# MiksuNy/rust_ray_tracing

Measured on AMD Instinct MI355X. Metric: Mray/s at 1920x1080, 8 spp, Sponza BVH; 1/2/4/8-GPU scaling + % HBM roofline, higher is better.
Workload: dtype f32

## Files before the change

include/mipt_diag.h:

```cpp
#ifndef MIPT_DIAG_H
#define MIPT_DIAG_H

#include <stdint.h>

#ifdef __cplusplus
extern "C" {
#endif

#if defined(__GNUC__)
#define MIPT_DIAG_API __attribute__((visibility("default")))
#else
#define MIPT_DIAG_API
#endif

MIPT_DIAG_API int mipt_debug_eval(int op, const float *a, const float *b, uint64_t n, float *out);

MIPT_DIAG_API int mipt_debug_eval_range(int op, uint32_t first_bits, uint64_t n, float y, float *out);

MIPT_DIAG_API int mipt_debug_wgsl(int op, const float *in, uint64_t n, const uint32_t *texels, uint32_t tex_w, uint32_t tex_h, float *out);

MIPT_DIAG_API int mipt_debug_texel(const float *uv, uint64_t n, const uint32_t *pool, uint64_t pool_words, uint32_t offset, uint32_t w, uint32_t h,
                                   float *rgb_out, uint64_t *clamped_out);

MIPT_DIAG_API int mipt_debug_divide(float *d_buf, uint64_t n_floats, float divisor, void *stream);
MIPT_DIAG_API int mipt_debug_popcount(const uint32_t *d_bitmap, uint64_t n_words, uint64_t *d_out, void *stream);

MIPT_DIAG_API int mipt_debug_tile_order(const uint32_t *cost, uint32_t n_tiles, uint32_t samples, uint32_t *order_out);
MIPT_DIAG_API int mipt_diag_scene_tile_order(const void *scene, uint32_t *cost_out, uint32_t *order_out, uint32_t cap, uint32_t info_out[3]);

MIPT_DIAG_API int mipt_debug_hot_select(const uint32_t *cost, uint32_t n_slots, uint32_t samples, uint32_t n_hot, uint32_t *hot_out, uint32_t *bits_out);
MIPT_DIAG_API int mipt_diag_scene_hot_pixels(const void *scene, uint32_t *pixel_cost_out, uint32_t cap_slots, uint32_t *hot_out, uint32_t cap_hot, uint32_t info_out[3]);

MIPT_DIAG_API const char *mipt_diag_last_error(void);

MIPT_DIAG_API int mipt_internal_pair_order(const void *nodes, uint32_t n_nodes, uint32_t *order_out, uint32_t cap, uint32_t *n_records_out);
MIPT_DIAG_API uint32_t mipt_internal_pair_order_top(void);
MIPT_DIAG_API int mipt_internal_tri_slots(const void *nodes, uint32_t n_nodes, uint32_t n_tris, uint32_t *slot_out, uint32_t *n_slots_out);

MIPT_DIAG_API int mipt_diag_scene_sizes(const void *scene, uint64_t out[2]);
MIPT_DIAG_API int mipt_diag_scene_tables(const void *scene, uint64_t out[3]);
MIPT_DIAG_API int mipt_diag_scene_read(const void *scene, int which, void *dst, uint64_t bytes);
MIPT_DIAG_API int mipt_diag_scene_hash(const void *scene, uint64_t out[2]);

MIPT_DIAG_API int mipt_diag_host_layout(const void *desc, uint8_t *geom_out, uint64_t geom_cap, uint8_t *attr_out, uint64_t attr_cap,
                                        uint64_t *sizes_out, uint32_t *info_out);

MIPT_DIAG_API int mipt_diag_hash_words(const void *words, uint64_t n_words, uint64_t *out);

MIPT_DIAG_API int mipt_diag_write_obj(const char *path, const void *tris, uint64_t n_tris, const char *mtllib, const char *const *material_names,
                                      uint32_t n_materials);

#ifdef __cplusplus
}
#endif
#endif
```

rust_ray_tracing_amd/_lib.py:

```python
from __future__ import annotations

import ctypes as C
import os

import numpy as np

_HERE = os.path.dirname(os.path.abspath(__file__))
LIB_PATH = os.environ.get("MIPT_LIB") or os.path.join(_HERE, "libmipt.so")

VERTEX = np.dtype([("position", "<f4", 3), ("tex_coord_x", "<f4"), ("normal", "<f4", 3), ("tex_coord_y", "<f4")])
TRIANGLE = np.dtype([("vertices", VERTEX, 3), ("material_id", "<u4"), ("_pad", "u1", 12)])
NODE = np.dtype([("bounds_min", "<f4", 3), ("first_tri_or_child", "<u4"), ("bounds_max", "<f4", 3), ("num_tris", "<u4")])
MATERIAL = np.dtype([
    ("base_color", "<f4", 3), ("transmission", "<f4"), ("specular_tint", "<f4", 3), ("ior", "<f4"),
    ("emission", "<f4", 3), ("roughness", "<f4"), ("metallic", "<f4"), ("transparency", "<f4"),
    ("base_color_tex_id", "<u4"), ("transparency_tex_id", "<u4"), ("roughness_tex_id", "<u4"),
    ("metallic_tex_id", "<u4"), ("emission_tex_id", "<u4"), ("normal_tex_id", "<u4")])
CAMERA = np.dtype([("look_at", "<f4", (4, 4)), ("position", "<f4", 3), ("_pad", "<f4")])
assert VERTEX.itemsize == 32 and TRIANGLE.itemsize == 112 and NODE.itemsize == 32
assert MATERIAL.itemsize == 80 and CAMERA.itemsize == 80

NO_TEXTURE = 0xFFFFFFFF

SEED_PIXEL_STREAM, SEED_PER_SAMPLE = 0, 1
# ... 348 lines not shown
    lib.mipt_temporal_history_bytes.argtypes = [u32, u32, u32]
    lib.mipt_temporal_history_bytes.restype = u64
    lib.mipt_temporal.argtypes = [to, vp, tb, C.c_int]
    lib.mipt_temporal.restype = C.c_int
    lib.mipt_temporal_device.argtypes = [to, vp, tb, vp]
    lib.mipt_temporal_device.restype = C.c_int
    vo, vb = C.POINTER(MiptVarianceOptions), C.POINTER(MiptVarianceBuffers)
    lib.mipt_denoise_variance_workspace_bytes.argtypes = [u32, u32, u32]
    lib.mipt_denoise_variance_workspace_bytes.restype = u64
    lib.mipt_denoise_variance.argtypes = [vo, vb, C.c_int]
    lib.mipt_denoise_variance.restype = C.c_int
    lib.mipt_denoise_variance_device.argtypes = [vo, vb, vp, u64, vp]
    lib.mipt_denoise_variance_device.restype = C.c_int
    uo, ub = C.POINTER(MiptUpsampleOptions), C.POINTER(MiptUpsampleBuffers)
    lib.mipt_upsample_workspace_bytes.argtypes = [u32, u32, u32, u32]
    lib.mipt_upsample_workspace_bytes.restype = u64
    lib.mipt_upsample.argtypes = [uo, ub, C.c_int]
    lib.mipt_upsample.restype = C.c_int
    lib.mipt_upsample_device.argtypes = [uo, ub, vp, u64, vp]
    lib.mipt_upsample_device.restype = C.c_int
    lib.mipt_render_adaptive.argtypes = [vp, vp, u32, C.POINTER(MiptOptions), vp, vp, vp, C.POINTER(MiptStats)]
    lib.mipt_render_adaptive.restype = C.c_int
    lib.mipt_render_adaptive_device.argtypes = [vp, vp, u32, C.POINTER(MiptOptions), vp, vp, vp, vp, C.POINTER(MiptStats)]
    lib.mipt_render_adaptive_device.restype = C.c_int
    so, sb = C.POINTER(MiptSampleMapOptions), C.POINTER(MiptSampleMapBuffers)
    lib.mipt_sample_map_workspace_bytes.argtypes = [u32, u32, u32]
    lib.mipt_sample_map_workspace_bytes.restype = u64
    lib.mipt_sample_map.argtypes = [so, sb, C.c_int]
    lib.mipt_sample_map.restype = C.c_int
    lib.mipt_sample_map_device.argtypes = [so, sb, vp, vp]
    lib.mipt_sample_map_device.restype = C.c_int
    return lib


MULTITEST_LIB_PATH = os.path.join(_HERE, "libmipt_multitest.so")
_multitest = None


def load_multitest() -> C.CDLL:
    global _multitest
    if _multitest is not None:
        return _multitest
    load()
    if not os.path.exists(MULTITEST_LIB_PATH):
        raise ImportError(f"{MULTITEST_LIB_PATH} is missing: run __graft_entry__.build()")
    lib = _bind(C.CDLL(MULTITEST_LIB_PATH))
    lib.rccl_double_inject.argtypes = [C.c_int, C.c_int]
    lib.rccl_double_inject.restype = C.c_longlong
    _multitest = lib
    return lib


DIAG_LIB_PATH = os.path.join(_HERE, "libmipt_diag.so")
DIAG_EXPORTS = ["mipt_debug_eval", "mipt_debug_eval_range", "mipt_debug_wgsl", "mipt_debug_texel", "mipt_debug_divide", "mipt_debug_popcount", "mipt_debug_tile_order", "mipt_diag_scene_tile_order", "mipt_debug_hot_select", "mipt_diag_scene_hot_pixels", "mipt_diag_last_error",
                "mipt_internal_pair_order", "mipt_internal_pair_order_top", "mipt_internal_tri_slots",
                "mipt_diag_scene_sizes", "mipt_diag_scene_tables", "mipt_diag_scene_read", "mipt_diag_scene_hash", "mipt_diag_write_obj", "mipt_diag_host_layout", "mipt_diag_hash_words"]
_diag = None


def load_diag() -> C.CDLL:
    global _diag
    if _diag is not None:
        return _diag
    load()
    if not os.path.exists(DIAG_LIB_PATH):
        raise ImportError(f"{DIAG_LIB_PATH} is missing: run __graft_entry__.build()")
    lib = C.CDLL(DIAG_LIB_PATH)
    vp = C.c_void_p
    lib.mipt_debug_eval.argtypes = [C.c_int, vp, vp, C.c_uint64, vp]
    lib.mipt_debug_eval.restype = C.c_int
    lib.mipt_debug_eval_range.argtypes = [C.c_int, C.c_uint32, C.c_uint64, C.c_float, vp]
    lib.mipt_debug_eval_range.restype = C.c_int
    lib.mipt_debug_wgsl.argtypes = [C.c_int, vp, C.c_uint64, vp, C.c_uint32, C.c_uint32, vp]
    lib.mipt_debug_wgsl.restype = C.c_int
    lib.mipt_debug_texel.argtypes = [vp, C.c_uint64, vp, C.c_uint64, C.c_uint32, C.c_uint32, C.c_uint32, vp, C.POINTER(C.c_uint64)]
    lib.mipt_debug_texel.restype = C.c_int
    lib.mipt_debug_divide.argtypes = [vp, C.c_uint64, C.c_float, vp]
    lib.mipt_debug_divide.restype = C.c_int
    lib.mipt_debug_popcount.argtypes = [vp, C.c_uint64, vp, vp]
    lib.mipt_debug_popcount.restype = C.c_int
    lib.mipt_debug_tile_order.argtypes = [vp, C.c_uint32, C.c_uint32, vp]
    lib.mipt_debug_tile_order.restype = C.c_int
    lib.mipt_diag_scene_tile_order.argtypes = [vp, vp, vp, C.c_uint32, C.POINTER(C.c_uint32 * 3)]
    lib.mipt_diag_scene_tile_order.restype = C.c_int
    lib.mipt_debug_hot_select.argtypes = [vp, C.c_uint32, C.c_uint32, C.c_uint32, vp, vp]
    lib.mipt_debug_hot_select.restype = C.c_int
    lib.mipt_diag_scene_hot_pixels.argtypes = [vp, vp, C.c_uint32, vp, C.c_uint32, C.POINTER(C.c_uint32 * 3)]
    lib.mipt_diag_scene_hot_pixels.restype = C.c_int
    lib.mipt_diag_last_error.argtypes = []
    lib.mipt_diag_last_error.restype = C.c_char_p
    u32p = C.POINTER(C.c_uint32)
    lib.mipt_internal_pair_order.argtypes = [vp, C.c_uint32, vp, C.c_uint32, u32p]
    lib.mipt_internal_pair_order.restype = C.c_int
    lib.mipt_internal_pair_order_top.argtypes = []
    lib.mipt_internal_pair_order_top.restype = C.c_uint32
    lib.mipt_internal_tri_slots.argtypes = [vp, C.c_uint32, C.c_uint32, vp, u32p]
    lib.mipt_internal_tri_slots.restype = C.c_int
    lib.mipt_diag_scene_sizes.argtypes = [vp, C.POINTER(C.c_uint64 * 2)]
    lib.mipt_diag_scene_sizes.restype = C.c_int
    lib.mipt_diag_scene_tables.argtypes = [vp, C.POINTER(C.c_uint64 * 3)]
    lib.mipt_diag_scene_tables.restype = C.c_int
    lib.mipt_diag_scene_read.argtypes = [vp, C.c_int, vp, C.c_uint64]
    lib.mipt_diag_scene_read.restype = C.c_int
    lib.mipt_diag_scene_hash.argtypes = [vp, C.POINTER(C.c_uint64 * 2)]
    lib.mipt_diag_scene_hash.restype = C.c_int
    lib.mipt_diag_write_obj.argtypes = [C.c_char_p, vp, C.c_uint64, C.c_char_p, C.POINTER(C.c_char_p), C.c_uint32]
    lib.mipt_diag_write_obj.restype = C.c_int
    lib.mipt_diag_host_layout.argtypes = [vp, vp, C.c_uint64, vp, C.c_uint64, C.POINTER(C.c_uint64 * 2), C.POINTER(C.c_uint32 * 4)]
    lib.mipt_diag_host_layout.restype = C.c_int
    lib.mipt_diag_hash_words.argtypes = [vp, C.c_uint64, C.POINTER(C.c_uint64)]
    lib.mipt_diag_hash_words.restype = C.c_int
    _diag = lib
    return lib


class MiptError(RuntimeError):
    def __init__(self, code: int, where: str):
        self.code = code
        msg = load().mipt_last_error()
        super().__init__(f"{where} failed with status {code}: {msg.decode() if msg else ''}")


def check(code: int, where: str) -> None:
    if code != 0:
        raise MiptError(code, where)


def ptr(a: np.ndarray) -> C.c_void_p:
    return C.c_void_p(a.ctypes.data)
```

rust_ray_tracing_amd/csrc/mipt_api.cpp:

```cpp
#include "../../include/mipt.h"
#include "pt_kernel.h"
#include "mipt_scene.h"

#include <atomic>
#include <chrono>
#include <cmath>
#include <cstdarg>
#include <cstdio>
#include <cstdlib>
#include <cstring>
#include <exception>
#include <memory>
#include <mutex>
#include <new>
#include <string>
#include <thread>
#include <vector>

static_assert(sizeof(MiptVec3) == 12, "Vec3f");
static_assert(sizeof(MiptVertex) == 32, "Vertex");
static_assert(sizeof(MiptTriangle) == 112 && offsetof(MiptTriangle, material_id) == 96, "Triangle");
static_assert(sizeof(MiptNode) == 32 && offsetof(MiptNode, first_tri_or_child) == 12 &&
                  offsetof(MiptNode, bounds_max) == 16 && offsetof(MiptNode, num_tris) == 28, "Node");
static_assert(sizeof(MiptMaterial) == 80 && offsetof(MiptMaterial, ior) == 28 && offsetof(MiptMaterial, emission) == 32 &&
// ... 397 lines not shown
    if (nodes_cap < scene->n_nodes) return fail(MIPT_ERR_INVALID_ARG, "mipt_scene_get_bvh: nodes_cap %u < %u nodes", nodes_cap, scene->n_nodes);
    MIPT_HIP(hipSetDevice(scene->device));
    MIPT_HIP(hipMemcpy(nodes_out, scene->d_nodes, (size_t)scene->n_nodes * sizeof(MiptNode), hipMemcpyDeviceToHost));
    if (tri_order_out) MIPT_HIP(hipMemcpy(tri_order_out, scene->d_tri_order, scene->n_tris * sizeof(uint32_t), hipMemcpyDeviceToHost));
    if (n_nodes_out) *n_nodes_out = scene->n_nodes;
    return MIPT_OK;
}

uint64_t mipt_packed_pixels(uint32_t width, uint32_t height, uint32_t tile_world) {
    if (tile_world == 0) tile_world = 1;
    const uint64_t tiles = (uint64_t)((width + 7u) / 8u) * ((height + 7u) / 8u);
    return ((tiles + tile_world - 1u) / tile_world) * 64ull;
}

static int validate_options(const MiptOptions *opt) {
    if (!opt) return fail(MIPT_ERR_INVALID_ARG, "options == NULL");
    if (opt->width == 0 || opt->height == 0) return fail(MIPT_ERR_INVALID_ARG, "Width and height must be greater than 0");
    if (opt->max_ray_depth == 0) return fail(MIPT_ERR_INVALID_ARG, "Max ray depth must be greater than 0");
    if (opt->samples == 0) return fail(MIPT_ERR_INVALID_ARG, "Sample count must be greater than 0");
    if ((uint64_t)opt->width * opt->height >= 2147483648ull - 87636354ull)
        return fail(MIPT_ERR_INVALID_ARG, "width*height too large for the reference's 32-bit pixel seed");
    if (opt->seed_mode > MIPT_SEED_PER_SAMPLE) return fail(MIPT_ERR_INVALID_ARG, "unknown seed_mode %u", opt->seed_mode);
    if (opt->traversal > MIPT_TRAVERSAL_CULLED) return fail(MIPT_ERR_INVALID_ARG, "unknown traversal %u", opt->traversal);
    const uint32_t world = opt->tile_world ? opt->tile_world : 1u;
    if (opt->tile_rank >= world) return fail(MIPT_ERR_INVALID_ARG, "tile_rank %u >= tile_world %u", opt->tile_rank, world);
    if ((opt->flags & MIPT_FLAG_SUM) && opt->seed_mode != MIPT_SEED_PER_SAMPLE && opt->sample_begin > 1)
        return fail(MIPT_ERR_INVALID_ARG, "sample_begin needs MIPT_SEED_PER_SAMPLE (the pixel stream cannot be entered mid-way)");
    if (opt->shading > MIPT_SHADING_WGPU) return fail(MIPT_ERR_INVALID_ARG, "unknown shading mode %u", opt->shading);
    if (!(opt->cull_margin >= 0.0f) || opt->cull_margin > 1.0f) return fail(MIPT_ERR_INVALID_ARG, "cull_margin must be in [0, 1]");
    for (uint32_t r : opt->reserved)
        if (r) return fail(MIPT_ERR_INVALID_ARG, "reserved option fields must be 0");
    return MIPT_OK;
}

static int validate_batch(const MiptScene *scene, const MiptCamera *cameras, uint32_t n_views, const MiptOptions *opt, const char *who) {
    if (!scene || !cameras) return fail(MIPT_ERR_INVALID_ARG, "%s: null scene or cameras", who);
    if (n_views == 0) return fail(MIPT_ERR_INVALID_ARG, "%s: n_views == 0", who);
    int rc = validate_options(opt);
    if (rc) return rc;
    if (opt->tile_world > 1) return fail(MIPT_ERR_INVALID_ARG, "%s: tile_world %u: a batch is not tile-sharded (0 or 1)", who, opt->tile_world);
    if (opt->flags & MIPT_FLAG_PACKED) return fail(MIPT_ERR_INVALID_ARG, "%s: MIPT_FLAG_PACKED: a batch is not tile-sharded", who);
    if ((uint64_t)n_views * opt->width * opt->height >= MIPT_BATCH_MAX_PIXELS)
        return fail(MIPT_ERR_INVALID_ARG, "%s: %u views of %ux%u: n_views*width*height must stay below 2^32", who, n_views, opt->width, opt->height);
    return MIPT_OK;
}

}
#ifndef MIPT_HOT_LANES_NUM
#define MIPT_HOT_LANES_NUM 2
#endif
#ifndef MIPT_HOT_LANES_DEN
#define MIPT_HOT_LANES_DEN 1
#endif
static int render_launch(MiptScene *scene, const MiptCamera *cameras, uint32_t n_views, bool batch, const MiptOptions *opt,
                         float *d_hdr_rgb, uint8_t *d_rgba8, void *hip_stream, MiptStats *stats, bool pack_single) {
    const char *who = batch ? "mipt_render_batch_device" : "mipt_render_device";
    int rc = MIPT_OK;
    if (batch) {
        if ((rc = validate_batch(scene, cameras, n_views, opt, who))) return rc;
    } else {
        if (!scene || !cameras) return fail(MIPT_ERR_INVALID_ARG, "mipt_render_device: null scene or camera");
        if ((rc = validate_options(opt))) return rc;
    }
    if (!d_hdr_rgb) return fail(MIPT_ERR_INVALID_ARG, "%s: d_hdr_rgb == NULL", who);
    const uint32_t world = opt->tile_world ? opt->tile_world : 1u;
    const bool packed = (opt->flags & MIPT_FLAG_PACKED) != 0 && (world > 1 || pack_single);
    if ((opt->flags & MIPT_FLAG_ACCUM) && !(opt->flags & MIPT_FLAG_SUM))
        return fail(MIPT_ERR_INVALID_ARG, "MIPT_FLAG_ACCUM needs MIPT_FLAG_SUM (a running sum, divided once at the end)");
    if (d_rgba8 && (packed || (opt->flags & MIPT_FLAG_SUM)))
        return fail(MIPT_ERR_INVALID_ARG, "RGBA8 output needs a full-frame mean buffer (not PACKED / SUM)");
    MIPT_HIP(hipSetDevice(scene->device));
    hipStream_t stream = (hipStream_t)hip_stream;
    const MiptCamera *camera = cameras;

    mipt::DevParams pr{};
    pr.width = opt->width; pr.height = opt->height; pr.samples = opt->samples; pr.max_depth = opt->max_ray_depth;
    pr.seed_mode = opt->shading == MIPT_SHADING_WGPU ? (uint32_t)MIPT_SEED_PER_SAMPLE : opt->seed_mode;
    pr.sample_begin = opt->sample_begin ? opt->sample_begin : 1u;
    pr.sum_only = (opt->flags & MIPT_FLAG_SUM) ? 1u : 0u;
    pr.packed = packed ? 1u : 0u;
    pr.accumulate = (opt->flags & MIPT_FLAG_ACCUM) ? 1u : 0u;
    pr.tile_rank = opt->tile_rank; pr.tile_world = world;
    pr.tiles_x = (opt->width + 7u) / 8u; pr.tiles_y = (opt->height + 7u) / 8u;
    const uint64_t tiles = (uint64_t)pr.tiles_x * pr.tiles_y;
    pr.n_local_tiles = (uint32_t)((tiles + world - 1u - opt->tile_rank) / world);
    pr.total_work = (unsigned long long)pr.n_local_tiles * 64ull * n_views;
    pr.aspect = (float)opt->width / (float)opt->height;
    pr.samples_f = (float)opt->samples;
    pr.cull_scale = 1.0f + opt->cull_margin;
    pr.service_num = 3; pr.service_den = 8; pr.reverse_tiles = 0;
    for (int c = 0; c < 3; c++)
        for (int r = 0; r < 3; r++) pr.cam[c * 3 + r] = camera->look_at[c][r];
    pr.cam[9] = camera->position.x; pr.cam[10] = camera->position.y; pr.cam[11] = camera->position.z;
    pr.hdr = d_hdr_rgb;
    pr.stats = scene->d_stats;

    const bool count = (opt->flags & MIPT_FLAG_COUNT) != 0;
    const bool cull = opt->traversal == MIPT_TRAVERSAL_CULLED;
    const int occ = mipt::trace_blocks_per_cu(batch, count, cull, (int)opt->shading);
    int bpc = occ;
    {
        const long long fit = (long long)(pr.total_work / (unsigned long long)(1.25 * scene->n_cu * mipt::kBlockThreads));
        const int cap = (int)(fit < 2 ? 2 : fit);
        if (cap < bpc) bpc = cap;
    }
    pr.leaf_period = (pr.total_work >= 4ull * (unsigned long long)scene->n_cu * (unsigned long long)occ * mipt::kBlockThreads) ? 4u : 1u;
    pr.leaf_den = 4u;
    int grid = 0;
    if ((rc = mipt::traversal_grid(scene, bpc, pr.total_work, &grid))) return rc;
    pr.ovf = scene->d_ovf;

    const bool touched = count && (opt->flags & MIPT_FLAG_TOUCHED) != 0 && opt->shading == 0;
    const size_t geom_lines = ((size_t)scene->dev.geom_bytes + 127) / 128, attr_lines = (scene->n_tris + 1) / 2;
    const size_t geom_words = (geom_lines + 31) / 32, attr_words = (attr_lines + 31) / 32;
    pr.touched = nullptr; pr.touched_attr_base = (uint32_t)(geom_words * 32);
    if (touched) {
        if (!scene->d_touched) MIPT_HIP(hipMalloc((void **)&scene->d_touched, (geom_words + attr_words) * sizeof(uint32_t)));
        MIPT_HIP(hipMemsetAsync(scene->d_touched, 0, (geom_words + attr_words) * sizeof(uint32_t), stream));
        pr.touched = scene->d_touched;
    }
    const bool order_on = !count && !batch && opt->shading == MIPT_SHADING_CPU && !(opt->flags & MIPT_FLAG_ACCUM) && pr.n_local_tiles != 0u &&
                          pr.n_local_tiles < (1u << 26);
    pr.tile_order = nullptr; pr.pixel_cost = nullptr; pr.hot = nullptr; pr.hot_bits = nullptr; pr.n_hot = 0u;
    const uint32_t n_slots = order_on ? pr.n_local_tiles * 64u : 0u;
    uint32_t hot_next = 0u;
    if (order_on) {
        const unsigned long long lanes = (unsigned long long)grid * mipt::kBlockThreads * MIPT_HOT_LANES_NUM / MIPT_HOT_LANES_DEN;
        hot_next = (uint32_t)(lanes < n_slots / 4u ? lanes : n_slots / 4u);
    }
    if (order_on) {
        const uint32_t key[7] = {opt->width, opt->height, world, opt->tile_rank, pr.n_local_tiles, pr.seed_mode, opt->samples};
        const size_t bytes = (size_t)pr.n_local_tiles * sizeof(uint32_t);
        const size_t hot_bytes = (size_t)(n_slots / 4u) * sizeof(uint32_t), work_bytes = mipt::hot_work_words(n_slots) * sizeof(uint32_t);
        if (scene->tile_cost_bytes < bytes || scene->tile_order_bytes < bytes || scene->pixel_cost_bytes < bytes * 64 || scene->hot_bytes < hot_bytes ||
            scene->hot_bits_bytes < bytes * 2 || scene->hot_work_bytes < work_bytes || memcmp(key, scene->tile_key, sizeof key) != 0 ||
            memcmp(pr.cam, scene->tile_cam, sizeof pr.cam) != 0)
            scene->tile_order_valid = false;
        if ((rc = mipt::grow_device_buffer((void **)&scene->d_tile_cost, &scene->tile_cost_bytes, bytes))) return rc;
        if ((rc = mipt::grow_device_buffer((void **)&scene->d_tile_order, &scene->tile_order_bytes, bytes))) return rc;
        if ((rc = mipt::grow_device_buffer((void **)&scene->d_pixel_cost, &scene->pixel_cost_bytes, bytes * 64))) return rc;
        if ((rc = mipt::grow_device_buffer((void **)&scene->d_hot, &scene->hot_bytes, hot_bytes))) return rc;
        if ((rc = mipt::grow_device_buffer((void **)&scene->d_hot_bits, &scene->hot_bits_bytes, bytes * 2))) return rc;
        if ((rc = mipt::grow_device_buffer((void **)&scene->d_hot_work, &scene->hot_work_bytes, work_bytes))) return rc;
        memcpy(scene->tile_key, key, sizeof key);
        memcpy(scene->tile_cam, pr.cam, sizeof pr.cam);
        MIPT_HIP(hipMemsetAsync(scene->d_pixel_cost, 0, bytes * 64, stream));
        pr.pixel_cost = scene->d_pixel_cost;
        pr.tile_order = scene->tile_order_valid ? scene->d_tile_order : nullptr;
        scene->tile_order_used = scene->tile_order_valid;
        scene->hot_used = 0u;
        if (scene->tile_order_valid && scene->hot_n != 0u) {
            pr.hot = scene->d_hot; pr.hot_bits = scene->d_hot_bits; pr.n_hot = scene->hot_n;
            pr.total_work += scene->hot_n;
            scene->hot_used = scene->hot_n;
        }
        scene->tile_order_valid = false;
    }
    mipt::DevBatch bt{};
    if (batch) {
        scene->h_cams.assign((size_t)n_views * 4, make_float4(0.0f, 0.0f, 0.0f, 0.0f));
        for (uint32_t v = 0; v < n_views; v++) {
            const MiptCamera &c = cameras[v];
            for (int col = 0; col < 3; col++) scene->h_cams[(size_t)v * 4 + col] = make_float4(c.look_at[col][0], c.look_at[col][1], c.look_at[col][2], 0.0f);
            scene->h_cams[(size_t)v * 4 + 3] = make_float4(c.position.x, c.position.y, c.position.z, 0.0f);
        }
        const size_t bytes = scene->h_cams.size() * sizeof(float4);
        if ((rc = mipt::grow_device_buffer((void **)&scene->d_cams, &scene->cams_bytes, bytes))) return rc;
        MIPT_HIP(hipMemcpyAsync(scene->d_cams, scene->h_cams.data(), bytes, hipMemcpyHostToDevice, stream));
        bt.cams = scene->d_cams;
        bt.view_pixels = opt->width * opt->height;
        bt.tiles_recip = 0xffffffffu / pr.n_local_tiles;
    }
    mipt::DevStats hs;
    float ms = 0.0f;
    rc = mipt::traversal_launch(
        scene, stream,
        [&]() -> int {
            MIPT_HIP(mipt::launch_trace(scene->dev, pr, batch ? &bt : nullptr, count, cull, (int)opt->shading, (int)grid, stream));
            return MIPT_OK;
        },
        [&]() -> int {
            if (order_on) {
                MIPT_HIP(mipt::launch_pixel_reduce(scene->d_pixel_cost, n_slots, opt->samples, scene->d_tile_cost, scene->d_hot_work, stream));
                MIPT_HIP(mipt::launch_tile_order(scene->d_tile_cost, pr.n_local_tiles, opt->samples, scene->d_tile_order, stream));
                if (hot_next != 0u)
                    MIPT_HIP(mipt::launch_hot_select(scene->d_pixel_cost, n_slots, opt->samples, hot_next, scene->d_hot_work, scene->d_hot, scene->d_hot_bits, stream));
                scene->hot_n = hot_next;
                scene->tile_order_valid = true;
            }
            if (touched) {
                MIPT_HIP(mipt::launch_popcount(scene->d_touched, geom_words, &scene->d_stats->touched_geom, stream));
                MIPT_HIP(mipt::launch_popcount(scene->d_touched + geom_words, attr_words, &scene->d_stats->touched_attr, stream));
            }
            if (d_rgba8) MIPT_HIP(mipt::launch_tonemap(d_hdr_rgb, (unsigned long long)opt->width * opt->height * n_views, 1.0f, d_rgba8, stream));
            return MIPT_OK;
        },
        hs, ms);
    if (rc && rc != MIPT_ERR_STACK) return rc;
    if (stats) {
        memset(stats, 0, sizeof *stats);
        stats->kernel_ms = ms;
        stats->rays = hs.rays; stats->inner_steps = hs.inner_steps; stats->tri_tests = hs.tri_tests;
        stats->hits = hs.hits; stats->texel_fetches = hs.texel_fetches; stats->stack_overflows = hs.stack_overflows;
        stats->tex_clamped = hs.tex_clamped; stats->max_stack = hs.max_stack; stats->pixels = hs.pixels;
        stats->diag[0] = hs.d_iters; stats->diag[1] = hs.d_inner_lanes; stats->diag[2] = hs.d_leaf_lanes;
        stats->diag[3] = hs.d_iters_inner; stats->diag[4] = hs.d_iters_leaf; stats->diag[5] = hs.d_services;
        stats->diag[6] = hs.d_service_lanes; stats->diag[7] = hs.d_cycles_service; stats->diag[8] = hs.d_cycles_total; stats->diag[9] = hs.d_cycles_mem; stats->diag[10] = hs.d_cycles_tail;
        stats->touched_lines[0] = hs.touched_geom; stats->touched_lines[1] = hs.touched_attr;
    }
    return rc;
}

int mipt::check_batch_args(const MiptScene *scene, const MiptCamera *cameras, uint32_t n_views, const MiptOptions *opt, const char *who) {
    return validate_batch(scene, cameras, n_views, opt, who);
}

int mipt::render_device_impl(MiptScene *scene, const MiptCamera *camera, const MiptOptions *opt,
                             float *d_hdr_rgb, uint8_t *d_rgba8, void *hip_stream, MiptStats *stats, bool pack_single) {
    return render_launch(scene, camera, 1u, false, opt, d_hdr_rgb, d_rgba8, hip_stream, stats, pack_single);
}

extern "C" {

int mipt_render_batch_device(MiptScene *scene, const MiptCamera *cameras, uint32_t n_views, const MiptOptions *opt,
                             float *d_hdr_rgb, uint8_t *d_rgba8, void *hip_stream, MiptStats *stats) {
    MIPT_NO_THROW(render_launch(scene, cameras, n_views, true, opt, d_hdr_rgb, d_rgba8, hip_stream, stats, false))
}

int mipt_render_batch(MiptScene *scene, const MiptCamera *cameras, uint32_t n_views, const MiptOptions *opt,
                      float *hdr_rgb, uint8_t *rgba8, MiptStats *stats) {
    int rc = validate_batch(scene, cameras, n_views, opt, "mipt_render_batch");
    if (rc) return rc;
    if (opt->flags & MIPT_FLAG_ACCUM) return fail(MIPT_ERR_INVALID_ARG, "MIPT_FLAG_ACCUM needs a caller-owned device buffer: use mipt_render_batch_device");
    if (rgba8 && (opt->flags & MIPT_FLAG_SUM))
        return fail(MIPT_ERR_INVALID_ARG, "RGBA8 output needs a full-frame mean buffer (not PACKED / SUM)");
    MIPT_HIP(hipSetDevice(scene->device));
    const uint64_t n_pix = (uint64_t)n_views * opt->width * opt->height;
    if ((rc = mipt::grow_device_buffer((void **)&scene->d_hdr, &scene->hdr_bytes, (size_t)n_pix * 3 * sizeof(float)))) return rc;
    uint8_t *d_rgba = nullptr;
    if (rgba8) {
// ... 88 lines not shown
```

rust_ray_tracing_amd/csrc/mipt_diag.hip:

```cpp
#include "../../include/mipt_diag.h"
#include "pt_device_math.h"
#include "pt_device_wgsl.h"
#include "pt_texel.h"
#include "mipt_host_util.h"
#include "pt_kernel.h"
#include "mipt_scene.h"

#include <stdio.h>

namespace {

thread_local char g_err[256] = "";

__global__ void debug_eval_kernel(int op, const float *__restrict__ a, const float *__restrict__ b, float b_scalar,
                                  unsigned long long n, float *__restrict__ out) {
    using namespace mipt;
    for (unsigned long long i = (unsigned long long)blockIdx.x * blockDim.x + threadIdx.x; i < n;
         i += (unsigned long long)gridDim.x * blockDim.x) {
        const float x = a[i], y = b ? b[i] : b_scalar;
        float r = 0.0f;
        switch (op) {
        case 0: r = gl_cosf(x); break;
        case 1: r = gl_log10f(x, GlTabGlobal()); break;
        case 2: r = gl_powf(x, y); break;
// ... 210 lines not shown
    return 0;
}

int mipt_diag_scene_tile_order(const void *scene, uint32_t *cost_out, uint32_t *order_out, uint32_t cap, uint32_t info_out[3]) {
    const MiptScene *s = (const MiptScene *)scene;
    if (!s || !info_out) { snprintf(g_err, sizeof g_err, "mipt_diag_scene_tile_order: bad argument"); return -1; }
    const uint32_t n = s->tile_order_valid ? s->tile_key[4] : 0u;
    info_out[0] = n; info_out[1] = s->tile_order_valid ? 1u : 0u; info_out[2] = s->tile_order_used ? 1u : 0u;
    if (n == 0u || !cost_out || !order_out) return 0;
    if (cap < n) { snprintf(g_err, sizeof g_err, "mipt_diag_scene_tile_order: cap %u < %u tiles", cap, n); return -1; }
    hipError_t e;
    if ((e = hipSetDevice(s->device)) != hipSuccess) return fail(e, "hipSetDevice");
    if ((e = hipMemcpy(cost_out, s->d_tile_cost, (size_t)n * 4, hipMemcpyDeviceToHost)) != hipSuccess) return fail(e, "hipMemcpy");
    if ((e = hipMemcpy(order_out, s->d_tile_order, (size_t)n * 4, hipMemcpyDeviceToHost)) != hipSuccess) return fail(e, "hipMemcpy");
    return 0;
}

int mipt_debug_hot_select(const uint32_t *cost, uint32_t n_slots, uint32_t samples, uint32_t n_hot, uint32_t *hot_out, uint32_t *bits_out) {
    if (!cost || !hot_out || !bits_out || n_slots == 0 || samples == 0 || n_hot == 0 || n_hot > n_slots) {
        snprintf(g_err, sizeof g_err, "mipt_debug_hot_select: bad argument");
        return -1;
    }
    const size_t bit_words = ((size_t)n_slots + 63) / 64 * 2;
    mipt::DevPtr<uint32_t> dcost, dwork, dhot, dbits;
    hipError_t e;
    if ((e = dcost.alloc(n_slots)) != hipSuccess) return fail(e, "hipMalloc");
    if ((e = dwork.alloc(mipt::hot_work_words(n_slots))) != hipSuccess) return fail(e, "hipMalloc");
    if ((e = dhot.alloc(n_hot)) != hipSuccess) return fail(e, "hipMalloc");
    if ((e = dbits.alloc(bit_words)) != hipSuccess) return fail(e, "hipMalloc");
    if ((e = hipMemcpy(dcost, cost, (size_t)n_slots * 4, hipMemcpyHostToDevice)) != hipSuccess) return fail(e, "hipMemcpy");
    if ((e = hipMemset(dhot, 0xff, (size_t)n_hot * 4)) != hipSuccess) return fail(e, "hipMemset");
    if ((e = hipMemset(dbits, 0xff, bit_words * 4)) != hipSuccess) return fail(e, "hipMemset");
    if ((e = mipt::launch_pixel_reduce(dcost, n_slots, samples, nullptr, dwork, nullptr)) != hipSuccess) return fail(e, "launch_pixel_reduce");
    if ((e = mipt::launch_hot_select(dcost, n_slots, samples, n_hot, dwork, dhot, dbits, nullptr)) != hipSuccess) return fail(e, "launch_hot_select");
    if ((e = hipMemcpy(hot_out, dhot, (size_t)n_hot * 4, hipMemcpyDeviceToHost)) != hipSuccess) return fail(e, "hipMemcpy");
    if ((e = hipMemcpy(bits_out, dbits, bit_words * 4, hipMemcpyDeviceToHost)) != hipSuccess) return fail(e, "hipMemcpy");
    return 0;
}

int mipt_diag_scene_hot_pixels(const void *scene, uint32_t *pixel_cost_out, uint32_t cap_slots, uint32_t *hot_out, uint32_t cap_hot, uint32_t info_out[3]) {
    const MiptScene *s = (const MiptScene *)scene;
    if (!s || !info_out) { snprintf(g_err, sizeof g_err, "mipt_diag_scene_hot_pixels: bad argument"); return -1; }
    const uint32_t n = s->tile_order_valid ? s->tile_key[4] * 64u : 0u, h = s->tile_order_valid ? s->hot_n : 0u;
    info_out[0] = n; info_out[1] = h; info_out[2] = s->tile_order_valid ? s->hot_used : 0u;
    if (n == 0u || !pixel_cost_out || !hot_out) return 0;
    if (cap_slots < n || cap_hot < h) { snprintf(g_err, sizeof g_err, "mipt_diag_scene_hot_pixels: cap %u / %u < %u slots / %u hot", cap_slots, cap_hot, n, h); return -1; }
    hipError_t e;
    if ((e = hipSetDevice(s->device)) != hipSuccess) return fail(e, "hipSetDevice");
    if ((e = hipMemcpy(pixel_cost_out, s->d_pixel_cost, (size_t)n * 4, hipMemcpyDeviceToHost)) != hipSuccess) return fail(e, "hipMemcpy");
    if (h != 0u && (e = hipMemcpy(hot_out, s->d_hot, (size_t)h * 4, hipMemcpyDeviceToHost)) != hipSuccess) return fail(e, "hipMemcpy");
    return 0;
}

int mipt_diag_scene_tables(const void *scene, uint64_t out[3]) {
    const MiptScene *s = (const MiptScene *)scene;
    if (!s || !out) { snprintf(g_err, sizeof g_err, "mipt_diag_scene_tables: bad argument"); return -1; }
    out[0] = s->n_texels * 4; out[1] = (uint64_t)s->dev.n_mats * sizeof(mipt::DevMaterial); out[2] = (uint64_t)s->dev.n_mats * sizeof(mipt::DevMaterialFull);
    return 0;
}

const char *mipt_diag_last_error(void) { return g_err; }

}
```

rust_ray_tracing_amd/csrc/mipt_scene.h:

```cpp
#pragma once
#include "../../include/mipt.h"
#include "mipt_host_util.h"
#include "pt_kernel.h"

#include <stddef.h>

#include <memory>
#include <vector>

namespace mipt { struct SceneMesh; }

struct MiptScene {
    int device = 0;
    mipt::DevScene dev{};
    void *d_geom = nullptr, *d_tri_attr = nullptr, *d_mats = nullptr, *d_mats_full = nullptr, *d_texels = nullptr;
    size_t geom_alloc = 0, attr_bytes = 0, mats_bytes = 0, mats_full_bytes = 0, texel_bytes = 0;
    uint64_t n_texels = 0;
    MiptNode *d_nodes = nullptr;
    uint32_t n_nodes = 0;
    uint32_t *d_tri_order = nullptr;
    MiptSceneInfo info{};
    mipt::DevStats *d_stats = nullptr;
    uint32_t *d_ovf = nullptr;
    size_t ovf_waves = 0;
    uint32_t *d_touched = nullptr;
    size_t n_tris = 0;
    float *d_hdr = nullptr;
    size_t hdr_bytes = 0;
    uint8_t *d_rgba = nullptr;
    size_t rgba_bytes = 0;
    float4 *d_cams = nullptr;
    size_t cams_bytes = 0;
    std::vector<float4> h_cams;
    uint32_t *d_tile_cost = nullptr, *d_tile_order = nullptr;
    size_t tile_cost_bytes = 0, tile_order_bytes = 0;
    uint32_t tile_key[7] = {0, 0, 0, 0, 0, 0, 0};
    float tile_cam[12] = {0};
    bool tile_order_valid = false;
    bool tile_order_used = false;
    uint32_t *d_pixel_cost = nullptr, *d_hot = nullptr, *d_hot_bits = nullptr, *d_hot_work = nullptr;
    size_t pixel_cost_bytes = 0, hot_bytes = 0, hot_bits_bytes = 0, hot_work_bytes = 0;
    uint32_t hot_n = 0;
    uint32_t hot_used = 0;
    void *d_qrays = nullptr, *d_qout = nullptr;
    size_t qrays_bytes = 0, qout_bytes = 0;
    hipEvent_t ev0 = nullptr, ev1 = nullptr;
    int n_cu = 0;
    uint32_t max_leaf = 0;
    uint32_t *d_refit_plan = nullptr, *d_refit_pair = nullptr;
    std::vector<uint32_t> refit_level_off;
    mipt::SceneMesh *mesh = nullptr;
};

namespace mipt {

void free_scene(MiptScene *s);
struct SceneDeleter { void operator()(MiptScene *s) const { free_scene(s); } };
using ScenePtr = std::unique_ptr<MiptScene, SceneDeleter>;
void free_mesh(MiptScene *s);
struct PartRec;
struct MeshMotionSource { const PartRec *prev_rec; const float *prev_pos; const uint32_t *idx; uint32_t n_parts, n_pos; };
bool mesh_motion_source(const MiptScene *s, MeshMotionSource *out);
int scene_finish_workspace(MiptScene *s);
int scene_clone_to(const MiptScene *src, int device, MiptScene **out);
int scene_clone_many(const MiptScene *src, const int *device_ids, int n_dev, MiptScene **outs);

struct MaterialTables {
    std::vector<DevMaterial> mats;
    std::vector<DevMaterialFull> mats_full;
    std::vector<uint32_t> texels;
    std::vector<uint32_t> tex_offset;
    uint64_t n_texels = 0;
};
int build_material_tables(const MiptSceneDesc *desc, MaterialTables *out, bool gather_texels = true);
int upload_material_tables(MiptScene *s, const MaterialTables &t);

struct ResidentBvh {
    DevPtr<MiptNode> d_nodes;
    uint32_t n_nodes = 0;
    DevPtr<uint32_t> d_tri_order;
    uint32_t levels = 0;
    double build_ms = 0.0;
};
int bvh_build_resident(const MiptTriangle *d_tris, uint32_t n_tris, int device_id, ResidentBvh *out);
void bvh_builder_resolve_kernels();

struct SceneGeometry {
    DevPtr<char> d_geom, d_tri_attr;
    size_t geom_alloc = 0, attr_bytes = 0, pairs_bytes = 0, pos_bytes = 0;
    DevPtr<MiptNode> d_nodes;
    DevPtr<uint32_t> d_tri_order;
    uint32_t n_tris = 0, n_nodes = 0, n_records_padded = 0, max_leaf = 0, tiny_axes = 0, root_a = 0, root_n = 0;
    double build_ms = 0.0, t_build = 0.0;
};
int build_geometry(const MiptTriangle *d_tris, uint32_t n_tris, uint32_t n_materials, int device_id, bool host_nodes, ResidentBvh *bvh,
                   SceneGeometry *out);
// ... 45 lines not shown
```

rust_ray_tracing_amd/csrc/pt_kernel.h:

```cpp
#pragma once
#include <hip/hip_runtime.h>
#include <stdint.h>

namespace mipt {

struct DevMaterial {
    float base[3]; uint32_t base_off;
    float emis[3]; uint32_t emis_off;
    uint32_t base_w, base_h, emis_w, emis_h;
    uint32_t pad[4];
};

struct DevMaterialFull {
    float base[3]; float transmission;
    float emission[3]; float ior;
    float roughness, metallic, transparency, pad0;
    uint32_t tex[6][3];
    uint32_t pad1[2];
};

struct DevScene {
    const float4 *pairs;
    const float4 *tri_pos;
    uint32_t tri_off_bytes, geom_bytes;
    uint32_t tiny_axes;
    const float4 *tri_attr;
    const DevMaterial *mats;
    const DevMaterialFull *mats_full;
    const uint32_t *texels;
    uint32_t n_pairs, n_tris, n_mats, n_texs;
    uint32_t root_a, root_n;
};

struct DevStats {
    unsigned long long queue;
    unsigned long long rays, inner_steps, tri_tests, hits, texel_fetches;
    unsigned long long stack_overflows, tex_clamped, max_stack, pixels;
    unsigned long long d_iters, d_inner_lanes, d_leaf_lanes, d_iters_inner, d_iters_leaf, d_services, d_service_lanes;
    unsigned long long d_cycles_service, d_cycles_total, d_cycles_mem, d_cycles_tail;
    unsigned long long touched_geom, touched_attr;
};

struct DevParams {
    uint32_t width, height, samples, max_depth;
    uint32_t seed_mode, sample_begin, sum_only, packed;
    uint32_t accumulate, pad1;
    uint32_t tile_rank, tile_world, tiles_x, tiles_y;
    uint32_t n_local_tiles;
    uint32_t n_hot;
    unsigned long long total_work;
    float aspect;
    float samples_f;
    float cull_scale;
    uint32_t reverse_tiles;
    uint32_t service_num, service_den;
    uint32_t leaf_period, leaf_den;
    float cam[12];
    float *hdr;
    uint32_t *ovf;
    DevStats *stats;
    const uint32_t *tile_order;
    uint32_t *pixel_cost;
    const uint32_t *hot;
    const uint32_t *hot_bits;
    uint32_t *touched;
    uint32_t touched_attr_base;
};

struct DevBatch {
    const float4 *cams;
    uint32_t view_pixels;
    uint32_t tiles_recip;
};

constexpr int kStackLds = 16;
constexpr int kStackOvf = 48;
constexpr int kWavesPerBlock = 4;
constexpr uint32_t kTriPosStride = 64;
constexpr int kBlockThreads = 64 * kWavesPerBlock;
constexpr uint32_t kMaxTris = 1u << 25;
constexpr uint32_t kMaxPairs = 1u << 24;

hipError_t launch_trace(const DevScene &sc, const DevParams &pr, const DevBatch *batch, bool count, bool cull, int shading,
                        int grid_blocks, hipStream_t stream);
int trace_blocks_per_cu(bool batch, bool count, bool cull, int shading);
hipError_t launch_trace_adaptive(const DevScene &sc, const DevParams &pr, const DevBatch &batch, const uint32_t *counts, bool count, bool cull,
                                 int shading, int grid_blocks, hipStream_t stream);
int trace_adaptive_blocks_per_cu(bool count, bool cull, int shading);
hipError_t launch_unpack_tiles(const float *packed_all, uint32_t width, uint32_t height,
                               uint32_t tile_world, float *hdr, hipStream_t stream);
hipError_t launch_tonemap(const float *hdr, unsigned long long n_pixels, float divisor,
                          uint8_t *rgba8, hipStream_t stream);

struct DevQuery {
    const float4 *rays;
    void *out;
    const uint32_t *tri_order;
    unsigned long long n_rays;
    float cull_scale;
    uint32_t *ovf;
    DevStats *stats;
};
// ... 111 lines not shown
```

rust_ray_tracing_amd/csrc/pt_kernel.hip:

```cpp
#include "pt_kernel.h"
#include "pt_device_math.h"
#include "pt_device_wgsl.h"
#include "pt_texel.h"
#include "pt_traverse.h"

namespace mipt {

namespace {

#ifndef MIPT_DIAG_STAMPS
#define MIPT_DIAG_STAMPS 0
#endif
constexpr bool DIAG_STAMPS = MIPT_DIAG_STAMPS != 0;

enum : uint32_t {
    ST_T = 0,
    ST_S = 1,
    ST_G = 2,
    ST_P = 3,
    ST_X = 4
};

__device__ __forceinline__ float min3_abs(float a, float b, float c) { float r; asm("v_min3_f32 %0, |%1|, |%2|, |%3|" : "=v"(r) : "v"(a), "v"(b), "v"(c)); return r; }

// ... 216 lines not shown
                    __builtin_amdgcn_wave_barrier();
                    if (scatter) {
                        const V3 rs = normalized(mk(dr[base], dr[base + 2u], dr[base + 4u]));
                        const V3 point = o + d * best_t;
                        const V3 new_dir = normalized(sc_normal + rs);
                        o = point + new_dir * 0.0001f;
                        d = new_dir;
                        bounces += 1;
                        path_done = !(bounces < pr.max_depth);
                    }
                }
            }
            if (state == ST_S) {
                if (path_done) {
                    if (!BATCH && pr.pixel_cost) atomicAdd(&pr.pixel_cost[slot], bounces + ((best_tri == kNoTri) ? 1u : 0u));
                    const V3 res = (bounces == 0u) ? incoming : incoming / (float)bounces;
                    final_color = final_color + res;
                    sample += 1;
                    uint32_t n_samples = pr.samples;
                    if (ADAPT) {
                        const uint32_t c = counts[view * bt.view_pixels + pix];
                        n_samples = c < pr.samples ? c : pr.samples;
                    }
                    if (sample < n_samples) {
                        state = ST_G;
                    } else {
                        if (!pr.sum_only) final_color = final_color / (ADAPT ? (float)n_samples : pr.samples_f);
                        float *dst = pr.hdr + (BATCH ? (size_t)view * bt.view_pixels + pix : (size_t)(pr.packed ? slot : pix)) * 3;
                        if (pr.accumulate) {
                            final_color = mk(dst[0] + final_color.x, dst[1] + final_color.y, dst[2] + final_color.z);
                        }
                        dst[0] = final_color.x; dst[1] = final_color.y; dst[2] = final_color.z;
                        c_pixels++;
                        state = ST_P;
                    }
                } else {
                    state = ST_T;
                    start_ray = true;
                }
            }
            {
                const unsigned long long m_p = __ballot(state == ST_P);
                if (m_p != 0ull) {
                    unsigned long long base = 0;
                    const uint32_t leader = (uint32_t)__ffsll((long long)m_p) - 1u;
                    if (lane == leader) base = atomicAdd(&pr.stats->queue, (unsigned long long)__popcll(m_p));
                    base = __shfl(base, (int)leader);
                    if (state == ST_P) {
                        const unsigned long long wi = base + lane_rank(m_p);
                        if (wi >= pr.total_work) {
                            state = ST_X;
                            if (COUNT && g_t_first_x == 0) g_t_first_x = clock64();
                        } else {
                            const bool is_hot = !BATCH && wi < (unsigned long long)pr.n_hot;
                            const unsigned long long wj = (BATCH || is_hot) ? wi : wi - pr.n_hot;
                            uint32_t lt = (uint32_t)(wj >> 6);
                            uint32_t p = (uint32_t)wj & 63u;
                            if (BATCH) {
                                const uint32_t n = pr.n_local_tiles;
                                uint32_t q = __umulhi(lt, bt.tiles_recip), r = lt - q * n;
                                if (r >= n) { q += 1u; r -= n; }
                                if (r >= n) { q += 1u; r -= n; }
                                view = q; lt = r;
                            }
                            uint32_t lt_o;
                            bool taken = false;
                            if (is_hot) {
                                const uint32_t s = pr.hot[(uint32_t)wi];
                                lt_o = s >> 6; p = s & 63u;
                            } else {
                                lt_o = (!BATCH && pr.tile_order) ? pr.tile_order[lt] : (pr.reverse_tiles ? (pr.n_local_tiles - 1u - lt) : lt);
                                if (!BATCH && pr.n_hot != 0u) taken = ((pr.hot_bits[lt_o * 2u + (p >> 5)] >> (p & 31u)) & 1u) != 0u;
                            }
                            const uint32_t gt = lt_o * pr.tile_world + pr.tile_rank;
                            const uint32_t px = (gt % pr.tiles_x) * 8u + (p & 7u);
                            const uint32_t py = (gt / pr.tiles_x) * 8u + (p >> 3);
                            if (px < pr.width && py < pr.height && !taken &&
                                (!ADAPT || counts[view * bt.view_pixels + py * pr.width + px] != 0u)) {
                                pix = py * pr.width + px;
                                if (!BATCH) slot = lt_o * 64u + p;
                                rng = 987612486u * (pix + 87636354u);
                                const uint32_t y = pr.height - py;
                                screen_x = ((((float)px / (float)pr.width) * 2.0f) - 1.0f) * pr.aspect;
                                screen_y = (((float)y / (float)pr.height) * 2.0f) - 1.0f;
                                final_color = mk(0.0f, 0.0f, 0.0f);
                                sample = 0;
                                state = ST_G;
                            }
                        }
                    }
                }
            }
            if (state == ST_G) {
                if (SHADING == 1 || pr.seed_mode != 0u) {
                    const uint32_t px = pix % pr.width, py = pix / pr.width;
                    rng = (pr.sample_begin + sample) * 6023u + (757283u * px + 872653746u * py);
                }
                const float jx = (rand_f32(rng) * 2.0f - 1.0f) * 0.0005f;
                const float jy = (rand_f32(rng) * 2.0f - 1.0f) * 0.0005f;
                const float rx = -screen_x + jx, ry = screen_y + jy, rz = 1.0f;
                if (BATCH) {
                    const float4 *cr = bt.cams + (size_t)view * 4;
                    const float4 c0 = cr[0], c1 = cr[1], c2 = cr[2], c3 = cr[3];
                    const V3 dir = mk(c0.x * rx + c1.x * ry + c2.x * rz,
                                      c0.y * rx + c1.y * ry + c2.y * rz,
                                      c0.z * rx + c1.z * ry + c2.z * rz);
                    d = normalized(dir);
                    o = mk(c3.x, c3.y, c3.z);
                } else {
                    const V3 dir = mk(pr.cam[0] * rx + pr.cam[3] * ry + pr.cam[6] * rz,
                                      pr.cam[1] * rx + pr.cam[4] * ry + pr.cam[7] * rz,
                                      pr.cam[2] * rx + pr.cam[5] * ry + pr.cam[8] * rz);
                    d = normalized(dir);
                    o = mk(pr.cam[9], pr.cam[10], pr.cam[11]);
                }
                ray_color = mk(1.0f, 1.0f, 1.0f);
                incoming = mk(0.0f, 0.0f, 0.0f);
                emitted = mk(0.0f, 0.0f, 0.0f);
                bounces = 0;
                if (SHADING == 1) prev_hit_point = o;
                state = ST_T;
                start_ray = true;
            }
            if (start_ray) {
                best_t = kMiss; best_u = 0.0f; best_v = 0.0f; best_tri = kNoTri;
// ... 452 lines not shown
```

Before: 2864.

## Schedule all pixels from a cost-sorted list instead of a hot prefix

```diff
diff --git a/include/mipt_diag.h b/include/mipt_diag.h
--- a/include/mipt_diag.h
+++ b/include/mipt_diag.h
@@ -30,6 +30,7 @@
 
 MIPT_DIAG_API int mipt_debug_hot_select(const uint32_t *cost, uint32_t n_slots, uint32_t samples, uint32_t n_hot, uint32_t *hot_out, uint32_t *bits_out);
 MIPT_DIAG_API int mipt_diag_scene_hot_pixels(const void *scene, uint32_t *pixel_cost_out, uint32_t cap_slots, uint32_t *hot_out, uint32_t cap_hot, uint32_t info_out[3]);
+MIPT_DIAG_API int mipt_diag_scene_list(const void *scene, uint32_t *list_out, uint32_t cap, uint32_t info_out[2]);
 
 MIPT_DIAG_API const char *mipt_diag_last_error(void);
 
diff --git a/rust_ray_tracing_amd/_lib.py b/rust_ray_tracing_amd/_lib.py
--- a/rust_ray_tracing_amd/_lib.py
+++ b/rust_ray_tracing_amd/_lib.py
@@ -424,7 +424,7 @@
 
 
 DIAG_LIB_PATH = os.path.join(_HERE, "libmipt_diag.so")
-DIAG_EXPORTS = ["mipt_debug_eval", "mipt_debug_eval_range", "mipt_debug_wgsl", "mipt_debug_texel", "mipt_debug_divide", "mipt_debug_popcount", "mipt_debug_tile_order", "mipt_diag_scene_tile_order", "mipt_debug_hot_select", "mipt_diag_scene_hot_pixels", "mipt_diag_last_error",
+DIAG_EXPORTS = ["mipt_debug_eval", "mipt_debug_eval_range", "mipt_debug_wgsl", "mipt_debug_texel", "mipt_debug_divide", "mipt_debug_popcount", "mipt_debug_tile_order", "mipt_diag_scene_tile_order", "mipt_debug_hot_select", "mipt_diag_scene_hot_pixels", "mipt_diag_scene_list", "mipt_diag_last_error",
                 "mipt_internal_pair_order", "mipt_internal_pair_order_top", "mipt_internal_tri_slots",
                 "mipt_diag_scene_sizes", "mipt_diag_scene_tables", "mipt_diag_scene_read", "mipt_diag_scene_hash", "mipt_diag_write_obj", "mipt_diag_host_layout", "mipt_diag_hash_words"]
 _diag = None
@@ -459,6 +459,8 @@
     lib.mipt_debug_hot_select.restype = C.c_int
     lib.mipt_diag_scene_hot_pixels.argtypes = [vp, vp, C.c_uint32, vp, C.c_uint32, C.POINTER(C.c_uint32 * 3)]
     lib.mipt_diag_scene_hot_pixels.restype = C.c_int
+    lib.mipt_diag_scene_list.argtypes = [vp, vp, C.c_uint32, C.POINTER(C.c_uint32 * 2)]
+    lib.mipt_diag_scene_list.restype = C.c_int
     lib.mipt_diag_last_error.argtypes = []
     lib.mipt_diag_last_error.restype = C.c_char_p
     u32p = C.POINTER(C.c_uint32)
diff --git a/rust_ray_tracing_amd/csrc/mipt_api.cpp b/rust_ray_tracing_amd/csrc/mipt_api.cpp
--- a/rust_ray_tracing_amd/csrc/mipt_api.cpp
+++ b/rust_ray_tracing_amd/csrc/mipt_api.cpp
@@ -473,6 +473,12 @@
 #ifndef MIPT_HOT_LANES_DEN
 #define MIPT_HOT_LANES_DEN 1
 #endif
+#ifndef MIPT_LIST_NUM
+#define MIPT_LIST_NUM 1
+#endif
+#ifndef MIPT_LIST_DEN
+#define MIPT_LIST_DEN 1
+#endif
 static int render_launch(MiptScene *scene, const MiptCamera *cameras, uint32_t n_views, bool batch, const MiptOptions *opt,
                          float *d_hdr_rgb, uint8_t *d_rgba8, void *hip_stream, MiptStats *stats, bool pack_single) {
     const char *who = batch ? "mipt_render_batch_device" : "mipt_render_device";
@@ -542,17 +548,19 @@
     }
     const bool order_on = !count && !batch && opt->shading == MIPT_SHADING_CPU && !(opt->flags & MIPT_FLAG_ACCUM) && pr.n_local_tiles != 0u &&
                           pr.n_local_tiles < (1u << 26);
-    pr.tile_order = nullptr; pr.pixel_cost = nullptr; pr.hot = nullptr; pr.hot_bits = nullptr; pr.n_hot = 0u;
+    pr.tile_order = nullptr; pr.pixel_cost = nullptr; pr.hot = nullptr; pr.hot_bits = nullptr; pr.n_list = 0u;
     const uint32_t n_slots = order_on ? pr.n_local_tiles * 64u : 0u;
-    uint32_t hot_next = 0u;
+    uint32_t hot_next = 0u, list_next = 0u;
     if (order_on) {
         const unsigned long long lanes = (unsigned long long)grid * mipt::kBlockThreads * MIPT_HOT_LANES_NUM / MIPT_HOT_LANES_DEN;
         hot_next = (uint32_t)(lanes < n_slots / 4u ? lanes : n_slots / 4u);
+        const uint32_t share = (uint32_t)((unsigned long long)n_slots * MIPT_LIST_NUM / MIPT_LIST_DEN);
+        list_next = hot_next == 0u ? 0u : (share > hot_next ? share : hot_next);
     }
     if (order_on) {
         const uint32_t key[7] = {opt->width, opt->height, world, opt->tile_rank, pr.n_local_tiles, pr.seed_mode, opt->samples};
         const size_t bytes = (size_t)pr.n_local_tiles * sizeof(uint32_t);
-        const size_t hot_bytes = (size_t)(n_slots / 4u) * sizeof(uint32_t), work_bytes = mipt::hot_work_words(n_slots) * sizeof(uint32_t);
+        const size_t hot_bytes = (size_t)n_slots * sizeof(uint32_t), work_bytes = mipt::hot_work_words(n_slots) * sizeof(uint32_t);
         if (scene->tile_cost_bytes < bytes || scene->tile_order_bytes < bytes || scene->pixel_cost_bytes < bytes * 64 || scene->hot_bytes < hot_bytes ||
             scene->hot_bits_bytes < bytes * 2 || scene->hot_work_bytes < work_bytes || memcmp(key, scene->tile_key, sizeof key) != 0 ||
             memcmp(pr.cam, scene->tile_cam, sizeof pr.cam) != 0)
@@ -569,11 +577,11 @@
         pr.pixel_cost = scene->d_pixel_cost;
         pr.tile_order = scene->tile_order_valid ? scene->d_tile_order : nullptr;
         scene->tile_order_used = scene->tile_order_valid;
-        scene->hot_used = 0u;
+        scene->hot_used = 0u; scene->list_used = 0u;
         if (scene->tile_order_valid && scene->hot_n != 0u) {
-            pr.hot = scene->d_hot; pr.hot_bits = scene->d_hot_bits; pr.n_hot = scene->hot_n;
-            pr.total_work += scene->hot_n;
-            scene->hot_used = scene->hot_n;
+            pr.hot = scene->d_hot; pr.hot_bits = scene->d_hot_bits; pr.n_list = scene->list_n;
+            if (scene->list_n == n_slots) pr.total_work = n_slots; else pr.total_work += scene->list_n;
+            scene->hot_used = scene->hot_n; scene->list_used = scene->list_n;
         }
         scene->tile_order_valid = false;
     }
@@ -604,9 +612,9 @@
             if (order_on) {
                 MIPT_HIP(mipt::launch_pixel_reduce(scene->d_pixel_cost, n_slots, opt->samples, scene->d_tile_cost, scene->d_hot_work, stream));
                 MIPT_HIP(mipt::launch_tile_order(scene->d_tile_cost, pr.n_local_tiles, opt->samples, scene->d_tile_order, stream));
-                if (hot_next != 0u)
-                    MIPT_HIP(mipt::launch_hot_select(scene->d_pixel_cost, n_slots, opt->samples, hot_next, scene->d_hot_work, scene->d_hot, scene->d_hot_bits, stream));
-                scene->hot_n = hot_next;
+                if (list_next != 0u)
+                    MIPT_HIP(mipt::launch_hot_select(scene->d_pixel_cost, n_slots, opt->samples, list_next, scene->d_hot_work, scene->d_hot, scene->d_hot_bits, stream));
+                scene->hot_n = hot_next; scene->list_n = list_next;
                 scene->tile_order_valid = true;
             }
             if (touched) {
diff --git a/rust_ray_tracing_amd/csrc/mipt_diag.hip b/rust_ray_tracing_amd/csrc/mipt_diag.hip
--- a/rust_ray_tracing_amd/csrc/mipt_diag.hip
+++ b/rust_ray_tracing_amd/csrc/mipt_diag.hip
@@ -286,6 +286,19 @@
     return 0;
 }
 
+int mipt_diag_scene_list(const void *scene, uint32_t *list_out, uint32_t cap, uint32_t info_out[2]) {
+    const MiptScene *s = (const MiptScene *)scene;
+    if (!s || !info_out) { snprintf(g_err, sizeof g_err, "mipt_diag_scene_list: bad argument"); return -1; }
+    const uint32_t n = s->tile_order_valid ? s->list_n : 0u;
+    info_out[0] = n; info_out[1] = s->tile_order_valid ? s->list_used : 0u;
+    if (n == 0u || !list_out) return 0;
+    if (cap < n) { snprintf(g_err, sizeof g_err, "mipt_diag_scene_list: cap %u < %u entries", cap, n); return -1; }
+    hipError_t e;
+    if ((e = hipSetDevice(s->device)) != hipSuccess) return fail(e, "hipSetDevice");
+    if ((e = hipMemcpy(list_out, s->d_hot, (size_t)n * 4, hipMemcpyDeviceToHost)) != hipSuccess) return fail(e, "hipMemcpy");
+    return 0;
+}
+
 int mipt_diag_scene_tables(const void *scene, uint64_t out[3]) {
     const MiptScene *s = (const MiptScene *)scene;
     if (!s || !out) { snprintf(g_err, sizeof g_err, "mipt_diag_scene_tables: bad argument"); return -1; }
diff --git a/rust_ray_tracing_amd/csrc/mipt_scene.h b/rust_ray_tracing_amd/csrc/mipt_scene.h
--- a/rust_ray_tracing_amd/csrc/mipt_scene.h
+++ b/rust_ray_tracing_amd/csrc/mipt_scene.h
@@ -42,6 +42,8 @@
     size_t pixel_cost_bytes = 0, hot_bytes = 0, hot_bits_bytes = 0, hot_work_bytes = 0;
     uint32_t hot_n = 0;
     uint32_t hot_used = 0;
+    uint32_t list_n = 0;
+    uint32_t list_used = 0;
     void *d_qrays = nullptr, *d_qout = nullptr;
     size_t qrays_bytes = 0, qout_bytes = 0;
     hipEvent_t ev0 = nullptr, ev1 = nullptr;
diff --git a/rust_ray_tracing_amd/csrc/pt_kernel.h b/rust_ray_tracing_amd/csrc/pt_kernel.h
--- a/rust_ray_tracing_amd/csrc/pt_kernel.h
+++ b/rust_ray_tracing_amd/csrc/pt_kernel.h
@@ -47,7 +47,7 @@
     uint32_t accumulate, pad1;
     uint32_t tile_rank, tile_world, tiles_x, tiles_y;
     uint32_t n_local_tiles;
-    uint32_t n_hot;
+    uint32_t n_list;
     unsigned long long total_work;
     float aspect;
     float samples_f;
diff --git a/rust_ray_tracing_amd/csrc/pt_kernel.hip b/rust_ray_tracing_amd/csrc/pt_kernel.hip
--- a/rust_ray_tracing_amd/csrc/pt_kernel.hip
+++ b/rust_ray_tracing_amd/csrc/pt_kernel.hip
@@ -292,8 +292,8 @@
                             state = ST_X;
                             if (COUNT && g_t_first_x == 0) g_t_first_x = clock64();
                         } else {
-                            const bool is_hot = !BATCH && wi < (unsigned long long)pr.n_hot;
-                            const unsigned long long wj = (BATCH || is_hot) ? wi : wi - pr.n_hot;
+                            const bool is_hot = !BATCH && wi < (unsigned long long)pr.n_list;
+                            const unsigned long long wj = (BATCH || is_hot) ? wi : wi - pr.n_list;
                             uint32_t lt = (uint32_t)(wj >> 6);
                             uint32_t p = (uint32_t)wj & 63u;
                             if (BATCH) {
@@ -310,7 +310,7 @@
                                 lt_o = s >> 6; p = s & 63u;
                             } else {
                                 lt_o = (!BATCH && pr.tile_order) ? pr.tile_order[lt] : (pr.reverse_tiles ? (pr.n_local_tiles - 1u - lt) : lt);
-                                if (!BATCH && pr.n_hot != 0u) taken = ((pr.hot_bits[lt_o * 2u + (p >> 5)] >> (p & 31u)) & 1u) != 0u;
+                                if (!BATCH && pr.n_list != 0u) taken = ((pr.hot_bits[lt_o * 2u + (p >> 5)] >> (p & 31u)) & 1u) != 0u;
                             }
                             const uint32_t gt = lt_o * pr.tile_world + pr.tile_rank;
                             const uint32_t px = (gt % pr.tiles_x) * 8u + (p & 7u);
```

New measurement: 3073, median of 6. 1.07x the previous value.
